# comprna/radian

Hardware: AMD Instinct MI355X
Metric: signal samples/s basecalled (chunk=1024, beam=10) (higher is better)
Workload: dtype f32

## Files before the change

### include/radian_hip.h

```cpp
#ifndef RADIAN_HIP_H
#define RADIAN_HIP_H

#include <stddef.h>
#include <stdint.h>

#ifdef __cplusplus
extern "C" {
#endif

#define RD_OK 0
#define RD_ERR_ARG (-1)
#define RD_ERR_HIP (-2)
#define RD_ERR_STATE (-3)
#define RD_ERR_NOMEM (-4)
#define RD_ERR_RCCL (-5)
#define RD_ERR_FORMAT (-6)
#define RD_ERR_IO (-7)
#define RD_LEN_MISSING_CONTEXT (-1)

typedef struct rd_ctx rd_ctx;

const char* rd_last_error(void);
int rd_version(void);
int rd_device_count(int* n);
int rd_decode_max_width(void);
int rd_decode_lane_width(void);

int rd_create(int device_id, rd_ctx** out);
int rd_destroy(rd_ctx* ctx);
int rd_sync(rd_ctx* ctx);
int rd_set_precision(rd_ctx* ctx, int mode);

typedef struct rd_weights_header {
    uint32_t magic;
    uint32_t version;
    uint32_t nb_filters;
    uint32_t kernel_size;
    uint32_t relu_units;
    uint32_t n_classes;
    uint32_t n_blocks;
    uint32_t dilations[16];
    uint32_t n_floats;
} rd_weights_header;
int rd_load_weights(rd_ctx* ctx, const void* blob, size_t nbytes);

int rd_load_lm(rd_ctx* ctx, const double* table, int k);
int rd_load_lm_absent(rd_ctx* ctx, int k);
int rd_load_lm_hashed(rd_ctx* ctx, const double* table, int table_order, int context_len);
int rd_set_logits(rd_ctx* ctx, int mode);
int rd_set_decode_partition(rd_ctx* ctx, int cus_per_xcd);
int rd_set_decode_math(rd_ctx* ctx, int mode);
int rd_set_head_pack(rd_ctx* ctx, int on);
int rd_head_pack_active(rd_ctx* ctx);
int64_t rd_head_pack_tiles(rd_ctx* ctx);
int rd_set_conv_slab(rd_ctx* ctx, int on);
int rd_conv_slab_active(rd_ctx* ctx);
int64_t rd_conv_slab_tiles(rd_ctx* ctx);

int rd_forward(rd_ctx* ctx, const float* windows, int n_windows, int chunk_len, float* probs);

int rd_assemble(rd_ctx* ctx, const float* probs, int n_windows, int chunk_len, int pad, int step, double* out,
                int64_t out_cap, int64_t* n_rows, int* is_f64);

int rd_decode_batch(rd_ctx* ctx, const void* probs, int prob_is_f64, const int64_t* seq_off, const int32_t* seq_len,
                    int n_seq, int beam_width, int use_lm, double s_thr, double r_thr, uint8_t* labels_out,
                    const int64_t* label_off, int32_t* label_len, double* best_score);

int rd_basecall_chunk(rd_ctx* ctx, const float* windows, int n_windows, int chunk_len, const int32_t* valid_len,
                      int beam_width, uint8_t* labels_out, int32_t* label_len);

int rd_basecall_global(rd_ctx* ctx, const float* windows, int chunk_len, int step, const int32_t* read_win_off,
                       const int32_t* pad, int n_reads, int beam_width, int use_lm, double s_thr, double r_thr,
                       uint8_t* labels_out, const int64_t* label_off, int32_t* label_len);

int rd_count_windows(int64_t n_samples, int chunk_len, int step);
int rd_basecall_reads_chunk(rd_ctx* ctx, const float* signal, const int64_t* read_off, int n_reads, int chunk_len,
                            int step, int beam_width, uint8_t* labels_out, int32_t* label_len);
int rd_basecall_reads_global(rd_ctx* ctx, const float* signal, const int64_t* read_off, int n_reads, int chunk_len,
                             int step, int beam_width, int use_lm, double s_thr, double r_thr, uint8_t* labels_out,
                             const int64_t* label_off, int32_t* label_len);

int rd_normalise_reads(rd_ctx* ctx, const int16_t* raw, const int64_t* read_off, int n_reads, int outlier_clip,
                       float* norm_out , int32_t* status);
int rd_basecall_raw_chunk(rd_ctx* ctx, const int16_t* raw, const int64_t* read_off, int n_reads, int outlier_clip,
                          int chunk_len, int step, int beam_width, uint8_t* labels_out, int32_t* label_len, int32_t* status);
int rd_basecall_raw_global(rd_ctx* ctx, const int16_t* raw, const int64_t* read_off, int n_reads, int outlier_clip,
                           int chunk_len, int step, int beam_width, int use_lm, double s_thr, double r_thr,
                           uint8_t* labels_out, const int64_t* label_off, int32_t* label_len, int32_t* status);

int rd_dev_alloc(rd_ctx* ctx, size_t bytes, void** d_ptr);
// ... 333 lines not shown
```

### radian_amd/_lib.py

```python
import ctypes
import os

HERE = os.path.dirname(os.path.abspath(__file__))
LIB_PATH = os.environ.get("RADIAN_HIP_LIB") or os.path.join(HERE, "libradian_hip.so")

c_i = ctypes.c_int
c_i32p = ctypes.POINTER(ctypes.c_int32)
c_i64 = ctypes.c_int64
c_i64p = ctypes.POINTER(ctypes.c_int64)
c_d = ctypes.c_double
c_dp = ctypes.POINTER(ctypes.c_double)
c_fp = ctypes.POINTER(ctypes.c_float)
c_u8p = ctypes.POINTER(ctypes.c_uint8)
c_u32 = ctypes.c_uint32
c_u64 = ctypes.c_uint64
c_vp = ctypes.c_void_p
c_sz = ctypes.c_size_t

SIGNATURES = {
    "rd_last_error": (ctypes.c_char_p, []),
    "rd_version": (c_i, []),
    "rd_device_count": (c_i, [ctypes.POINTER(c_i)]),
    "rd_decode_max_width": (c_i, []),
    "rd_decode_lane_width": (c_i, []),
    "rd_create": (c_i, [c_i, ctypes.POINTER(c_vp)]),
    "rd_destroy": (c_i, [c_vp]),
    "rd_sync": (c_i, [c_vp]),
    "rd_set_precision": (c_i, [c_vp, c_i]),
    "rd_load_weights": (c_i, [c_vp, c_vp, c_sz]),
    "rd_load_lm": (c_i, [c_vp, c_vp, c_i]),
    "rd_load_lm_absent": (c_i, [c_vp, c_i]),
    "rd_load_lm_hashed": (c_i, [c_vp, c_vp, c_i, c_i]),
    "rd_set_logits": (c_i, [c_vp, c_i]),
    "rd_set_decode_math": (c_i, [c_vp, c_i]),
    "rd_set_head_pack": (c_i, [c_vp, c_i]),
    "rd_head_pack_active": (c_i, [c_vp]),
    "rd_head_pack_tiles": (c_i64, [c_vp]),
    "rd_set_conv_slab": (c_i, [c_vp, c_i]),
    "rd_conv_slab_active": (c_i, [c_vp]),
    "rd_conv_slab_tiles": (c_i64, [c_vp]),
    "rd_set_decode_partition": (c_i, [c_vp, c_i]),
    "rd_forward": (c_i, [c_vp, c_vp, c_i, c_i, c_vp]),
    "rd_assemble": (c_i, [c_vp, c_vp, c_i, c_i, c_i, c_i, c_vp, c_i64, c_i64p, ctypes.POINTER(c_i)]),
    "rd_decode_batch": (c_i, [c_vp, c_vp, c_i, c_vp, c_vp, c_i, c_i, c_i, c_d, c_d, c_vp, c_vp, c_vp, c_vp]),
    "rd_basecall_chunk": (c_i, [c_vp, c_vp, c_i, c_i, c_vp, c_i, c_vp, c_vp]),
    "rd_basecall_global": (c_i, [c_vp, c_vp, c_i, c_i, c_vp, c_vp, c_i, c_i, c_i, c_d, c_d, c_vp, c_vp, c_vp]),
    "rd_count_windows": (c_i, [c_i64, c_i, c_i]),
    "rd_basecall_reads_chunk": (c_i, [c_vp, c_vp, c_vp, c_i, c_i, c_i, c_i, c_vp, c_vp]),
    "rd_basecall_reads_global": (c_i, [c_vp, c_vp, c_vp, c_i, c_i, c_i, c_i, c_i, c_d, c_d, c_vp, c_vp, c_vp]),
    "rd_basecall_reads_chunk_resident": (c_i, [c_vp, c_vp, c_vp, c_i, c_i, c_i, c_i, c_vp, c_vp]),
    "rd_basecall_reads_global_resident": (c_i, [c_vp, c_vp, c_vp, c_i, c_i, c_i, c_i, c_i, c_d, c_d, c_vp, c_vp, c_vp]),
    "rd_pipe_submit_reads": (c_i, [c_vp, c_vp, c_vp, c_i, c_i, c_i, c_i, c_vp, c_vp]),
    "rd_pipe_submit_reads_global": (c_i, [c_vp, c_vp, c_vp, c_i, c_i, c_i, c_i, c_i, c_d, c_d, c_vp, c_vp, c_vp]),
    "rd_pipe_submit_raw_global": (c_i, [c_vp, c_vp, c_vp, c_i, c_i, c_i, c_i, c_i, c_i, c_d, c_d, c_vp, c_vp, c_vp, c_vp]),
    "rd_pipe_submit_raw_chunk": (c_i, [c_vp, c_vp, c_vp, c_i, c_i, c_i, c_i, c_i, c_vp, c_vp, c_vp]),
    "rd_pipe_progress": (c_i, [c_vp, c_i64, c_i64p]),
    "rd_pipe_submitted": (c_i, [c_vp, c_i64p]),
    "rd_normalise_reads": (c_i, [c_vp, c_vp, c_vp, c_i, c_i, c_vp, c_vp]),
    "rd_basecall_raw_chunk": (c_i, [c_vp, c_vp, c_vp, c_i, c_i, c_i, c_i, c_i, c_vp, c_vp, c_vp]),
    "rd_basecall_raw_global": (c_i, [c_vp, c_vp, c_vp, c_i, c_i, c_i, c_i, c_i, c_i, c_d, c_d, c_vp, c_vp, c_vp, c_vp]),
    "rd_stitch_chunk": (c_i, [c_vp, c_vp, c_i, c_vp, c_i, c_vp, c_vp, c_vp, c_i]),
    "rd_fast5_open": (c_i, [ctypes.c_char_p, ctypes.POINTER(c_vp)]),
    "rd_fast5_open_mem": (c_i, [c_vp, c_sz, ctypes.POINTER(c_vp)]),
    "rd_fast5_close": (None, [c_vp]),
    "rd_fast5_count": (c_i, [c_vp, c_i64p]),
    "rd_fast5_lengths": (c_i, [c_vp, c_i64, c_i64, c_vp]),
    "rd_fast5_read_batch": (c_i, [c_vp, c_i64, c_i64, c_vp, c_i64, c_vp, c_vp, c_i]),
    "rd_lm_json_probe": (c_i, [c_vp, ctypes.c_size_t, ctypes.POINTER(c_i)]),
    "rd_lm_json_fill": (c_i, [c_vp, ctypes.c_size_t, c_i, c_vp, ctypes.POINTER(ctypes.c_int64), ctypes.POINTER(ctypes.c_int64)]),
    "rd_lm_json_write": (c_i, [ctypes.c_char_p, c_vp, c_i, c_i64p, c_i64p]),
    "rd_fasta_scan": (c_i, [c_vp, c_sz, c_i, ctypes.c_char_p, c_vp, c_vp, c_vp]),
    "rd_lm_build": (c_i, [c_vp, c_vp, c_vp, c_i64, c_i, c_i, c_i, c_d, c_d, c_i64, c_vp, c_vp, c_vp]),
    "rd_lm_score": (c_i, [c_vp, c_vp, c_vp, c_i64, c_i, c_d, c_i64, c_vp, c_dp]),
# ... 132 lines not shown
```

### radian_amd/backend.py

```python
import ctypes

import numpy as np

from . import _lib
from .weights import pack_blob, DEFAULT_DILATIONS

RD_TIMER_CONV, RD_TIMER_DECODE, RD_TIMER_HEAD, RD_TIMER_IN = 0, 1, 2, 3


class RadianHipError(RuntimeError):
    pass


def lib_path():
    return _lib.LIB_PATH


def _p(a):
    return None if a is None else a.ctypes.data_as(ctypes.c_void_p)


MISSING_CONTEXT = -1


# ... 972 lines not shown
            raise ValueError(f"LM table must be [4^{table_order},4], got {table.shape}")
        self._check(self._L.rd_load_lm_hashed(self._h, _p(table), int(table_order), int(context_len)))
        self.lm_k = context_len

    def set_logits(self, mode):
        self._check(self._L.rd_set_logits(self._h, {"f32": 0, "f16": 1}[mode] if isinstance(mode, str) else int(mode)))

    def set_trie_budget(self, nbytes):
        self._check(self._L.rd_set_trie_budget(self._h, int(nbytes)))

    def set_conv_fuse(self, on):
        self._check(self._L.rd_set_conv_fuse(self._h, 1 if on else 0))

    def set_head_pack(self, on):
        self._check(self._L.rd_set_head_pack(self._h, 1 if on else 0))

    def head_pack_active(self):
        return bool(self._L.rd_head_pack_active(self._h))

    def head_pack_tiles(self):
        return int(self._L.rd_head_pack_tiles(self._h))

    def set_conv_slab(self, on):
        self._check(self._L.rd_set_conv_slab(self._h, 1 if on else 0))

    def conv_slab_active(self):
        return bool(self._L.rd_conv_slab_active(self._h))

    def conv_slab_tiles(self):
        return int(self._L.rd_conv_slab_tiles(self._h))

    def set_decode_form(self, form):
        self._check(self._L.rd_set_decode_form(self._h, {"auto": 0, "waves": 1, "lanes": 2, "two": 3, "one": 4, "queue": 5}[form] if isinstance(form, str) else int(form)))

    def set_decode_partition(self, cus_per_xcd):
        self._check(self._L.rd_set_decode_partition(self._h, int(cus_per_xcd)))

    def set_decode_math(self, mode):
        self._check(self._L.rd_set_decode_math(self._h, {"fast": 0, "glibc": 1}[mode] if isinstance(mode, str) else int(mode)))

    def forward(self, windows):
        windows = np.ascontiguousarray(windows, dtype=np.float32)
        if windows.ndim != 2:
            raise ValueError("windows must be [n_windows, chunk_len]")
        n, T = windows.shape
        probs = np.empty((n, T, 5), dtype=np.float32)
        self._check(self._L.rd_forward(self._h, _p(windows), n, T, _p(probs)))
        return probs

    def assemble(self, probs, pad, step):
        probs = np.ascontiguousarray(probs, dtype=np.float32)
        nW, T, _ = probs.shape
        cap = (nW - 1) * step + T
        out = np.empty((max(cap, 1), 5), dtype=np.float64)
        n_rows = ctypes.c_int64(0)
        is64 = ctypes.c_int(0)
        self._check(self._L.rd_assemble(self._h, _p(probs), nW, T, int(pad), int(step), _p(out), out.shape[0],
                                        ctypes.byref(n_rows), ctypes.byref(is64)))
        out = out[: n_rows.value]
        return out if is64.value else out.astype(np.float32)

    def forward_reads(self, signals, chunk_len, step):
        flat, off = self._pack_reads(signals)
        nws = [self.count_windows(off[r + 1] - off[r], chunk_len, step) for r in range(len(signals))]
        tot = int(sum(nws))
        out = np.zeros((tot, chunk_len, 5), dtype=np.float32)
# ... 790 lines not shown
```

### radian_amd/csrc/common.h

```cpp
#pragma once
#include <hip/hip_runtime.h>
#include <stdint.h>
#include <stddef.h>
#include <string>
#include <vector>

#include "carve.h"
#include "polya_rules.h"

#define RD_OK 0
#define RD_ERR_ARG (-1)
#define RD_ERR_HIP (-2)
#define RD_ERR_STATE (-3)
#define RD_ERR_NOMEM (-4)
#define RD_ERR_RCCL (-5)

void rd_set_error(const char* fmt, ...);

#define RD_HIP(expr)                                                                                   \
    do {                                                                                               \
        hipError_t _e = (expr);                                                                        \
        if (_e != hipSuccess) {                                                                        \
            rd_set_error("%s:%d: %s failed: %s", __FILE__, __LINE__, #expr, hipGetErrorString(_e));   \
            return RD_ERR_HIP;                                                                         \
// ... 127 lines not shown
struct TileLists {
    const TileDesc* d[RD_MAX_LAYERS];
    int n[RD_MAX_LAYERS];
    int64_t rows[RD_MAX_LAYERS];
    const TileDesc* head_segs[RD_MAX_LAYERS];
    PackLayer pack[RD_MAX_LAYERS];
    int slab[RD_MAX_LAYERS];
    int slab_stream[RD_MAX_LAYERS];
};

struct KernelTimer {
    bool enabled = false;
    std::vector<hipEvent_t> starts, stops;
    size_t used = 0;
    double flops = 0.0;
    double bytes = 0.0;
    std::vector<double> each_flops;
    std::vector<int> each_tag;
};

constexpr int RD_MAX_LANES = 4;
struct FwdLane {
    hipStream_t st = nullptr;
    DevBuf act[3];
    hipEvent_t done = nullptr;
};

struct rd_ctx {
    int device = 0;
    int n_cu = 256;
    int precision = 0;
    int decode_form = 0;
    int decode_math = 1;
    int conv_fuse = 1;
    int64_t packed_tiles = 0;
    int head_pack = 1;
    int conv_slab = 1;
    int64_t slab_tiles = 0;
    int conv_shape = 0;
    int logits_f16 = 0;
    hipStream_t stream = nullptr;
    hipStream_t stream_hi = nullptr;
    hipEvent_t ev_chain = nullptr;
    Model model;
    LM lm;
    DevBuf ws_tiles, ws_raw;
    int tiles_nW = -1, tiles_T = -1;
    int tiles_slab = 0;
    FwdLane lanes[2 * RD_MAX_LANES];
    int part_mode = -1;
    int part_cus = 0;
    DevBuf ws_in, ws_probs, ws_mat, ws_seq, ws_nodes_child, ws_nodes_back, ws_labels, ws_misc;
    DevBuf ws_queue;
    DevBuf ws_wide, ws_wide_slot;
    DevBuf ws_align;
    DevBuf ws_ctc;
    DevBuf ws_calign;
    DevBuf ws_events, ws_events_io;
    DevBuf ws_polya, ws_polya_io;
    DevBuf ws_segment;
    DevBuf ws_sim;
    DevBuf ws_eval, ws_eval_model;
    DevBuf ws_site;
    DevBuf ws_quant;
    DevBuf pileup_sites;
    DevBuf pileup_profile;
    DevBuf ws_pileup;
    int64_t pileup_n_sites = -1;
    int64_t pileup_pairs = 0;
    int64_t trie_budget = (int64_t)24 << 30;
    void* h_stage = nullptr;
    size_t h_stage_cap = 0;
    bool h_stage_busy = false;
    KernelTimer timer_conv, timer_decode, timer_head, timer_in;
    void* rccl = nullptr;
    void* rpipe = nullptr;
    int pipe_group = 4;
    int pipe_lanes = 2;
    void* plan_cache[2] = {nullptr, nullptr};
    void* train = nullptr;
    void* map = nullptr;
};

size_t rd_model_image_floats(int nblocks);
void rd_model_bind(Model& m);
int rd_model_refresh_split(rd_ctx* ctx);
// ... 102 lines not shown
```

### radian_amd/csrc/context.hip

```cpp
#include "common.h"
#include "budget.h"
#include "../../include/radian_hip.h"
#include "../../include/radian_hip_diag.h"

#include <algorithm>
#include <stdarg.h>
#include <stdio.h>
#include <string.h>

static thread_local char g_err[1024] = "";

void rd_set_error(const char* fmt, ...)
{
    va_list ap;
    va_start(ap, fmt);
    vsnprintf(g_err, sizeof(g_err), fmt, ap);
    va_end(ap);
}

extern "C" const char* rd_last_error(void) { return g_err; }
extern "C" int rd_version(void) { return 1; }

int DevBuf::reserve(size_t bytes)
{
// ... 131 lines not shown
    t.starts.clear();
    t.stops.clear();
    t.each_flops.clear();
    t.each_tag.clear();
    t.used = 0;
    t.enabled = false;
}

extern "C" int rd_destroy(rd_ctx* ctx)
{
    if (!ctx) return RD_OK;
    (void)hipSetDevice(ctx->device);
    if (ctx->stream) (void)hipStreamSynchronize(ctx->stream);
    rd_rccl_finalize(ctx);
    rd_rpipe_destroy(ctx);
    rd_plan_cache_destroy_internal(ctx);
    rd_train_destroy(ctx);
    rd_map_destroy(ctx);
    timer_free(ctx->timer_conv);
    timer_free(ctx->timer_decode);
    timer_free(ctx->timer_head);
    timer_free(ctx->timer_in);
    for (int i = 0; i < 2 * RD_MAX_LANES; i++) {
        FwdLane& L = ctx->lanes[i];
        if (i > 0 && L.st) {
            (void)hipStreamSynchronize(L.st);
            if (i >= RD_MAX_LANES) rd_masked_stream_release(L.st);
            else (void)hipStreamDestroy(L.st);
        }
        if (L.done) (void)hipEventDestroy(L.done);
        for (DevBuf& b : L.act) b.release();
    }
    DevBuf* bufs[] = {&ctx->ws_tiles, &ctx->ws_raw, &ctx->ws_in, &ctx->ws_probs, &ctx->ws_mat, &ctx->ws_seq,
                      &ctx->ws_nodes_child, &ctx->ws_nodes_back, &ctx->ws_wide, &ctx->ws_wide_slot, &ctx->ws_align, &ctx->ws_ctc, &ctx->ws_calign, &ctx->ws_events, &ctx->ws_events_io, &ctx->ws_polya, &ctx->ws_polya_io, &ctx->ws_segment, &ctx->ws_eval, &ctx->ws_eval_model, &ctx->ws_site, &ctx->ws_quant, &ctx->pileup_sites, &ctx->pileup_profile, &ctx->ws_pileup, &ctx->ws_sim, &ctx->ws_queue, &ctx->ws_labels, &ctx->ws_misc, &ctx->model.storage,
                      &ctx->lm.storage, &ctx->lm.gate_storage};
    for (DevBuf* b : bufs) b->release();
    if (ctx->h_stage) (void)hipHostFree(ctx->h_stage);
    if (ctx->stream_hi) {
        (void)hipStreamSynchronize(ctx->stream_hi);
        (void)hipStreamDestroy(ctx->stream_hi);
    }
    if (ctx->ev_chain) (void)hipEventDestroy(ctx->ev_chain);
    if (ctx->stream) (void)hipStreamDestroy(ctx->stream);
    delete ctx;
    return RD_OK;
}

extern "C" int rd_set_precision(rd_ctx* ctx, int mode)
{
    RD_REQUIRE(ctx, "rd_set_precision: null context");
    RD_REQUIRE(mode >= 0 && mode <= 2, "rd_set_precision: mode %d (0 = fp32 MFMA, 1 = split-f16 f16x3, 2 = three-term bf16x3)", mode);
    ctx->precision = mode;
    return RD_OK;
}

extern "C" int rd_sync(rd_ctx* ctx)
{
    RD_REQUIRE(ctx, "rd_sync: null context");
    return rd_sync_lanes(ctx);
}

extern "C" int rd_set_logits(rd_ctx* ctx, int mode)
{
    RD_REQUIRE(ctx, "rd_set_logits: null context");
    RD_REQUIRE(mode == 0 || mode == 1, "rd_set_logits: mode %d (0 = float32 rows, 1 = float16 rows)", mode);
    ctx->logits_f16 = mode;
    return RD_OK;
}

extern "C" int rd_set_decode_form(rd_ctx* ctx, int form)
{
    RD_REQUIRE(ctx, "rd_set_decode_form: null context");
    RD_REQUIRE(form >= 0 && form <= 5, "rd_set_decode_form: form %d (0 = per launch, 1 = waves per sequence, 2 = candidates per lane, 3 = W <= 12: two sequences per "
               "wave, 4 = one, 5 = work queue)", form);
    ctx->decode_form = form;
    return RD_OK;
}

extern "C" int rd_set_trie_budget(rd_ctx* ctx, int64_t bytes)
{
    RD_REQUIRE(ctx, "rd_set_trie_budget: null context");
    RD_REQUIRE(bytes >= 0, "rd_set_trie_budget: negative budget");
    ctx->trie_budget = bytes ? bytes : (int64_t)24 << 30;
    return RD_OK;
}

extern "C" int rd_set_conv_shape(rd_ctx* ctx, int shape)
{
    RD_REQUIRE(ctx, "rd_set_conv_shape: null context");
    RD_REQUIRE(shape == 0 || shape == 1, "rd_set_conv_shape: shape %d (0 = 128-row tiles, two workgroups per CU; 1 = 256-row tiles, one workgroup per CU)", shape);
    ctx->conv_shape = shape;
    return RD_OK;
}

extern "C" int rd_set_conv_fuse(rd_ctx* ctx, int on)
{
    RD_REQUIRE(ctx, "rd_set_conv_fuse: null context");
    RD_REQUIRE(on == 0 || on == 1, "rd_set_conv_fuse: %d (1 = block 0's first conv inside its second, 0 = its own kernel)", on);
    ctx->conv_fuse = on;
    return RD_OK;
}

extern "C" int rd_set_head_pack(rd_ctx* ctx, int on)
{
    RD_REQUIRE(ctx, "rd_set_head_pack: null context");
    RD_REQUIRE(on == 0 || on == 1, "rd_set_head_pack: %d (1 = window heads as packed classes without their zero-padding taps, 0 = as head tiles)", on);
    ctx->head_pack = on;
    return RD_OK;
// ... 160 lines not shown
```

### radian_amd/csrc/decode.hip

```cpp
#include "common.h"
#include "glibc_math.h"
#include "glibc_tables.h"

#include <math.h>
#include <stdlib.h>

#include "decode_common.h"

namespace {

struct __attribute__((aligned(16))) Beam {
    double ptot, pb;
    double pnb;
    int last, len;
    int node;
    unsigned hist;
    unsigned hprev;
    int pad1;
    int child[4];
};
static_assert(sizeof(Beam) == 64, "Beam is one 64-B LDS record");

template <int R, int NW>
struct Cfg {
// ... 2 lines not shown
};
template <>
struct Cfg<2, 4> {
    static constexpr int WM = 64;
};


template <int NW>
__device__ __forceinline__ void seq_sync()
{
    if constexpr (NW == 1) {
        wave_sync();
    } else {
        __builtin_amdgcn_fence(__ATOMIC_RELEASE, "wavefront");
        asm volatile("s_waitcnt lgkmcnt(0)\n\ts_barrier" ::: "memory");
        __builtin_amdgcn_fence(__ATOMIC_ACQUIRE, "wavefront");
    }
}

template <typename PT, int R, int NW, bool LM, bool HC, bool GX>
__device__ __forceinline__ void beam_search_body(const DecodeArgs& a, const int seq)
{
    static_assert(LM || !HC, "hashed contexts only exist with an LM");
    constexpr int WM = Cfg<R, NW>::WM;
    constexpr int TPB = 64 * NW;
    constexpr int NS = R * NW;
    constexpr int KG = R == 1 ? 16 : 4;
    constexpr int SEG = 64 + KG;
    constexpr int HB = (WM + 63) / 64;
    constexpr int LOG_TN = WM > 128 ? 12 : WM > 64 ? 11 : R * NW <= 2 ? 9 : 10;
    constexpr int TN = 1 << LOG_TN;
    constexpr int SB = WM > 128 ? 9 : 8;
    constexpr int SMASK = (1 << SB) - 1;
    static_assert(WM <= 64 * HB && HB <= 4 && WM <= 256, "the kept beams fit the lanes of one wave, up to four times; a table entry holds a slot in 8 bits");
    static_assert(HB == 1 || !HC, "hashed contexts exist for up to 64 beams");
    const int tid = threadIdx.x;
    const int lane = tid & 63;
    const int wv = NW == 1 ? 0 : __builtin_amdgcn_readfirstlane(tid >> 6);
    const int T = a.seq_len[seq];
    const PT* __restrict__ probs = (const PT*)a.probs;
    const int64_t row_a = a.seq_off[seq];
    const int64_t row_b = a.seq_off2 ? a.seq_off2[seq] : row_a;
    const int split = a.seq_off2 ? a.seq_split[seq] : 0;
    int4* __restrict__ childtab = a.childtab + a.node_off[seq];
    int* __restrict__ backptr = a.backptr + a.node_off[seq];
    const int W = a.W;
    const unsigned ctx_mask = LM ? ((a.k >= 16) ? 0xffffffffu : ((1u << (2 * a.k)) - 1u)) : 0u;

    __shared__ Beam st[2][WM];
    constexpr int SCR = 5 * WM, KEYS = NS * SEG;
    __shared__ __attribute__((aligned(16))) double dbuf[NW == 1 ? (SCR > KEYS ? SCR : KEYS) : SCR + KEYS + (SCR & 1)];
    double* const cpy_pnb = dbuf;
    double* const cpy_pb = dbuf + WM;
    double* const mb_v = dbuf + 2 * WM;
    double* const mP = dbuf + 3 * WM;
    double* const mQ = dbuf + 4 * WM;
    double* const keyC = NW == 1 ? dbuf : dbuf + SCR + (SCR & 1);
    __shared__ int mb_q[WM];
    __shared__ int d_sel[WM], newslot[WM];
    __shared__ unsigned claims[WM];
    __shared__ double lp[64][5];
    __shared__ double praw[LM ? 64 : 1][5];
    __shared__ double sent[LM ? 64 : 1];
    __shared__ int seg_s[NS], seg_v[NS], mflag[NW];
    __shared__ unsigned tab[TN];
    constexpr bool GXL = GX && R == 1;
    __shared__ uint64_t gx_lds[GXL ? 256 : 1];
    if constexpr (GXL)
        for (int i = tid; i < 256; i += TPB) gx_lds[i] = g_gm_exp_tab[i];
    const uint64_t* const gx_exp = GXL ? gx_lds : g_gm_exp_tab;
    __shared__ __attribute__((aligned(16))) unsigned ring[2][HC ? WM : 1][16];

    for (int i = tid; i < TN; i += TPB) tab[i] = i == 0 ? 0u : 0xffffffffu;
    if (tid == 0) {
        Beam& b = st[0][0];
        b.ptot = 0.0;
        b.pb = 0.0;
        b.pnb = -INFINITY;
        b.last = -1;
        b.len = 0;
        b.node = 0;
        b.hist = 0u;
        b.hprev = 0u;
        b.pad1 = 0;
        for (int c = 0; c < 4; c++) b.child[c] = 0;
        childtab[0] = make_int4(0, 0, 0, 0);
        backptr[0] = 0;
    }
    int nb = 1;
    int next_id = 1;
    int cur = 0;
    bool missed = false;
    seq_sync<NW>();

    for (int t0 = 0; t0 < T; t0 += 64) {
        if (NW == 1 || wv == 0) {
            const int t = t0 + lane;
            if (t < T) {
                const PT* __restrict__ prow = probs + ((t < split ? row_a : row_b) + t) * 5;
                double s4 = 0.0;
#pragma unroll 1
                for (int c = 0; c < 5; c++) {
                    const double pc = (double)prow[c];
                    lp[lane][c] = safe_log<GX>(pc);
                    if constexpr (LM) {
                        praw[lane][c] = pc;
                        if (c < 4) s4 = c == 0 ? pc : s4 + pc;
                    }
                }
                if constexpr (LM) {
                    const double s = s4;
                    double ent = 0.0;
                    bool any = false;
#pragma unroll 1
                    for (int c = 0; c < 4; c++) {
                        const double pc = praw[lane][c];
                        double n;
                        if (s == 0.0) n = pc;
                        else if constexpr (sizeof(PT) == 4) n = (double)((float)pc / (float)s);
                        else n = pc / s;
                        if (n > 0) {
                            double v = n * log_m<GX>(n);
                            ent = any ? ent + v : v;
                            any = true;
                        }
                    }
                    sent[lane] = any ? -ent : 0.0;
                }
            }
        }
        seq_sync<NW>();

        const int tend = (T - t0) < 64 ? (T - t0) : 64;
        for (int tt = 0; tt < tend; tt++) {
            const Beam* os = st[cur];
            Beam* __restrict__ ns = st[cur ^ 1];
            const int ncand = 5 * nb;

            bool valid[R], is_copy[R];
            int bi[R], kk[R], pj[R], dcopy[R], xch[R];
            double c_ptot[R], c_pnb[R], c_pb[R];
            const double lp_blank = lp[tt][4];
            bool s_open = false;
            if constexpr (LM) s_open = __builtin_amdgcn_readfirstlane((int)(sent[tt] > a.s_thr)) != 0;
            const double ptot_last = os[nb - 1].ptot;
            int myn[HB];
            if constexpr (HB == 1) {
                myn[0] = os[lane < nb ? lane : 0].node;
            } else {
#pragma unroll
                for (int h = 0; h < HB; h++) myn[h] = os[lane + 64 * h < nb ? lane + 64 * h : 0].node;
            }
            double2 pp[R];
            double pnb_i[R];
            int2 ll[R];
            int chx[R];
#pragma unroll
            for (int s = 0; s < R; s++) {
                const int q = s * TPB + tid;
                valid[s] = q < ncand;
                const int i = valid[s] ? q / 5 : 0;
                const int k = q - 5 * (q / 5);
                bi[s] = i;
                kk[s] = k;
                is_copy[s] = k == 0;
                pp[s] = *(const double2*)&os[i].ptot;
                pnb_i[s] = os[i].pnb;
                ll[s] = *(const int2*)&os[i].last;
                int4 c4 = *(const int4*)&os[i].child[0];
                asm("" : "+v"(c4.x), "+v"(c4.y), "+v"(c4.z), "+v"(c4.w));
// ... 85 lines not shown
#pragma unroll
                    for (int s = 0; s < R; s++)
                        if (xch[s] != 0 && nj == xch[s]) pj[s] = j;
                }
            }
            bool any_merge = false;
#pragma unroll
            for (int s = 0; s < R; s++) any_merge |= __any(pj[s] >= 0);
            if constexpr (NW > 1) {
                if (lane == 0) mflag[wv] = any_merge ? 1 : 0;
            }
            seq_sync<NW>();
            if constexpr (NW > 1) {
                int m = 0;
#pragma unroll
                for (int w = 0; w < NW; w++) m |= mflag[w];
                any_merge = __builtin_amdgcn_readfirstlane(m) != 0;
            }

#pragma unroll
            for (int s = 0; s < R; s++) {
                const bool mext = pj[s] >= 0;
                const double cp = cpy_pnb[mext ? pj[s] : 0];
                const double x = mext ? cp : c_pb[s];
                const double y = mext ? c_ptot[s] : c_pnb[s];
                const double r = GX ? lae_gx(x, y, gx_exp) : lae(x, y);
                c_ptot[s] = is_copy[s] ? r : c_ptot[s];
                if (mext) {
                    mb_q[pj[s]] = s * TPB + tid;
                    mb_v[pj[s]] = c_ptot[s];
                    mQ[pj[s]] = r;
                }
            }
            if (any_merge) {
                seq_sync<NW>();
#pragma unroll
                for (int s = 0; s < R; s++) {
                    const int qe = mb_q[bi[s]];
                    const double mv = mb_v[bi[s]];
                    const bool m = valid[s] & is_copy[s] & (qe >= 0);
                    const double r = GX ? lae_gx(c_ptot[s], m ? mv : -INFINITY, gx_exp) : lae(c_ptot[s], m ? mv : -INFINITY);
                    if (m) mP[bi[s]] = r;
                }
                seq_sync<NW>();
#pragma unroll
                for (int s = 0; s < R; s++) {
                    const int q = s * TPB + tid;
                    const int j = is_copy[s] ? bi[s] : (pj[s] >= 0 ? pj[s] : 0);
                    const int qe = mb_q[j];
                    const double P = mP[j], Q = mQ[j], cb = cpy_pb[j];
                    const bool merged = valid[s] & (is_copy[s] ? qe >= 0 : pj[s] >= 0);
                    const int qother = is_copy[s] ? qe : 5 * j;
                    const bool mk = merged & (q < qother);
                    const bool mke = mk & !is_copy[s];
                    c_ptot[s] = mk ? P : c_ptot[s];
                    c_pnb[s] = mk ? Q : c_pnb[s];
                    c_pb[s] = mke ? cb : c_pb[s];
                    dcopy[s] = mke ? j : dcopy[s];
                    valid[s] = valid[s] & (!merged | mk);
                }
            }

            double key[R];
            bool surv[R];
            int lidx[R], scnt[R], vcnt[R];
            const double tau = (nb == W) ? ptot_last + lp_blank : -INFINITY;
#pragma unroll
            for (int s = 0; s < R; s++) {
                key[s] = valid[s] ? c_ptot[s] : __builtin_nan("");
                surv[s] = valid[s] && key[s] >= tau;
                const unsigned long long mv = __ballot(valid[s]), ms = __ballot(surv[s]);
                vcnt[s] = __popcll(mv);
                scnt[s] = __popcll(ms);
                lidx[s] = (int)__builtin_amdgcn_mbcnt_hi((unsigned)(ms >> 32), __builtin_amdgcn_mbcnt_lo((unsigned)ms, 0u));
                double* kseg = keyC + (s * NW + wv) * SEG;
                if (lane < KG) kseg[scnt[s] + lane] = -INFINITY;
                if (surv[s]) kseg[lidx[s]] = key[s];
                if constexpr (NW > 1) {
                    if (lane == 0) {
                        seg_s[s * NW + wv] = scnt[s];
                        seg_v[s * NW + wv] = vcnt[s];
                    }
                }
            }
            seq_sync<NW>();
            int segn[NS];
            int nvalid = 0;
#pragma unroll
            for (int g = 0; g < NS; g++) {
                if constexpr (NW > 1) {
                    segn[g] = __builtin_amdgcn_readfirstlane(seg_s[g]);
                    nvalid += __builtin_amdgcn_readfirstlane(seg_v[g]);
                } else {
                    segn[g] = scnt[g];
                    nvalid += vcnt[g];
                }
            }
            int rank[R];
#pragma unroll
            for (int s = 0; s < R; s++) rank[s] = 0;
#pragma unroll
            for (int g = 0; g < NS; g++) {
                const double* kseg = keyC + g * SEG;
                for (int j = 0; j < segn[g]; j += KG) {
                    double2 kq[KG / 2];
#pragma unroll
                    for (int u = 0; u < KG / 2; u++) kq[u] = *(const double2*)&kseg[j + 2 * u];
#pragma unroll
                    for (int u = 0; u < KG / 4; u++)
#pragma unroll
                        for (int s = 0; s < R; s++)
                            rank[s] = count4_gt(rank[s], kq[2 * u].x, kq[2 * u].y, kq[2 * u + 1].x, kq[2 * u + 1].y, key[s]);
                }
            }
            const int nb_new = nvalid < W ? nvalid : W;

            if constexpr (NW == 1 && R == 1) {
                const bool top = surv[0] && rank[0] < W;
                const unsigned long long m_top = __ballot(top), m_same = __ballot(top && dcopy[0] >= 0 && rank[0] == dcopy[0]);
                if (m_top == m_same && __popcll(m_top) == nb && nb_new == nb) {
                    if (top) {
                        Beam* const here = st[cur] + rank[0];
                        *(double2*)&here->ptot = make_double2(c_ptot[0], c_pb[0]);
                        here->pnb = c_pnb[0];
                    }
                    wave_sync();
                    continue;
                }
            }

            auto scatter = [&]() {
#pragma unroll
                for (int s = 0; s < R; s++) {
                    if (surv[s] && rank[s] < W) {
                        const int r = rank[s];
                        *(double2*)&ns[r].ptot = make_double2(c_ptot[s], c_pb[s]);
                        ns[r].pnb = c_pnb[s];
                        d_sel[r] = (dcopy[s] & SMASK) | (bi[s] << SB) | (kk[s] << (2 * SB));
                        atomicAdd(&claims[r], 1u);
                        if (dcopy[s] >= 0) newslot[dcopy[s]] = r;
                    }
                }
            };
            scatter();
            seq_sync<NW>();
            unsigned n_claims[HB], my_tn2[HB];
            int sel[HB], my_newslot[HB];
            bool claim_bad;
            if constexpr (HB == 1) {
                n_claims[0] = claims[lane < nb_new ? lane : 0];
                sel[0] = d_sel[lane < nb_new ? lane : 0];
                my_newslot[0] = newslot[lane < nb ? lane : 0];
                my_tn2[0] = tab[myn[0] & (TN - 1)];
                asm volatile("" : "+v"(sel[0]), "+v"(my_newslot[0]), "+v"(my_tn2[0]));
                claim_bad = (lane < nb_new) & (n_claims[0] != 1u);
            } else {
                claim_bad = false;
// ... 144 lines not shown
                                ch.x = __hip_atomic_load(cp + 0, __ATOMIC_RELAXED, __HIP_MEMORY_SCOPE_AGENT);
                                ch.y = __hip_atomic_load(cp + 1, __ATOMIC_RELAXED, __HIP_MEMORY_SCOPE_AGENT);
                                ch.z = __hip_atomic_load(cp + 2, __ATOMIC_RELAXED, __HIP_MEMORY_SCOPE_AGENT);
                                ch.w = __hip_atomic_load(cp + 3, __ATOMIC_RELAXED, __HIP_MEMORY_SCOPE_AGENT);
                            }
                            asm volatile("s_waitcnt vmcnt(0)" : "+v"(ch.x), "+v"(ch.y), "+v"(ch.z), "+v"(ch.w));
                        }
                        if (act) {
                            const int new_node = is_ext ? my_node : meta.x;
                            *(int2*)&ns[bl].last = make_int2(is_ext ? cl : sl2.x, is_ext ? sl2.y + 1 : sl2.y);
                            const unsigned h_new = ((unsigned)meta.y << 2) | (unsigned)cl;
                            if constexpr (LM) {
                                if (a.lm_missing && is_ext && sl2.y + 1 >= a.k && t0 + tt + 1 < T) {
                                    const unsigned cx = h_new & ctx_mask;
                                    missed |= ((a.lm_missing[cx >> 5] >> (cx & 31)) & 1u) != 0u;
                                }
                            }
                            *(int4*)&ns[bl].node = make_int4(new_node, is_ext ? (int)h_new : meta.y, meta.z, 0);
                            *(int4*)&ns[bl].child[0] = make_int4(is_ext ? ch.x : chs.x, is_ext ? ch.y : chs.y, is_ext ? ch.z : chs.z, is_ext ? ch.w : chs.w);
                            tab[new_node & (TN - 1)] = (((unsigned)new_node >> LOG_TN) << 8) | (unsigned)bl;
                        }
                        fresh_h[h] = fresh;
                        ps_h[h] = ps;
                        cl_h[h] = cl;
                        node_h[h] = my_node;
                    }
#pragma unroll
                    for (int h = 0; h < HB; h++)
                        if (fresh_h[h] && ps_h[h] >= 0) ns[ps_h[h]].child[cl_h[h]] = node_h[h];
                }
            }
            nb = nb_new;
            cur ^= 1;
            seq_sync<NW>();
        }
    }

    int tid_end = tid;
    asm volatile("" : "+v"(tid_end));
    const bool any_missed = LM && __any(missed);
    if (tid_end == 0) {
        __builtin_amdgcn_s_waitcnt(0);
        const char* ka = (const char*)__builtin_amdgcn_kernarg_segment_ptr();
        asm volatile("" : "+s"(ka));
        const DecodeArgs* ap = (const DecodeArgs*)ka;
        const Beam& fs = st[cur][0];
        int n = fs.node;
        const int len = fs.len;
        uint8_t* out = ap->labels + ap->label_off[seq];
        for (int p = len - 1; p >= 0; p--) {
            const int bp = __hip_atomic_load(&backptr[n], __ATOMIC_RELAXED, __HIP_MEMORY_SCOPE_AGENT);
            out[p] = (uint8_t)(bp & 3);
            n = bp >> 2;
        }
        ap->label_len[seq] = any_missed ? -1 : len;
        if (ap->best_score) ap->best_score[seq] = fs.ptot;
    }
}


template <typename PT, int R, int NW, bool LM, bool HC, bool GX>
__global__ __launch_bounds__(64 * NW) void beam_search_kernel(DecodeArgs a)
{
    beam_search_body<PT, R, NW, LM, HC, GX>(a, (int)blockIdx.x);
}

template <typename PT, int R, int NW, bool LM, bool HC, bool GX>
__global__ __launch_bounds__(64 * NW) void beam_search_queue_kernel(DecodeArgs a, int n_seq, int* counter)
{
    __shared__ int s_next;
    for (;;) {
        if (threadIdx.x == 0) s_next = atomicAdd(counter, 1);
        __syncthreads();
        const int seq = __builtin_amdgcn_readfirstlane(s_next);
        __syncthreads();
        if (seq >= n_seq) return;
        beam_search_body<PT, R, NW, LM, HC, GX>(a, seq);
        __syncthreads();
    }
}


template <typename PT, bool LM, bool GX, int R>
__global__ __launch_bounds__(64) void beam_search2_kernel(DecodeArgs a, int n_seq)
{
    constexpr int WM = R == 1 ? 6 : 12;
    constexpr int TS = 32;
    constexpr int KG = R == 1 ? 16 : 8;
    constexpr int SEG = 32 + KG;
// ... 583 lines not shown
        if (!ctx->lm.loaded) {
            rd_set_error("decode with use_lm=1 but no LM table loaded (rd_load_lm)");
            return RD_ERR_STATE;
        }
        int rc = ensure_lm_gate(ctx, r_thr, st);
        if (rc) return rc;
    }
    if (ctx->ws_nodes_child.reserve((size_t)total_nodes * sizeof(int4))) return RD_ERR_NOMEM;
    if (ctx->ws_nodes_back.reserve((size_t)total_nodes * sizeof(int))) return RD_ERR_NOMEM;
    DecodeArgs a;
    a.probs = d_probs;
    a.seq_off = d_seq_off;
    a.seq_off2 = d_seq_off2;
    a.seq_split = d_seq_split;
    a.seq_len = d_seq_len;
    a.node_off = d_node_off;
    a.label_off = d_label_off;
    a.W = W;
    a.glibc_math = ctx->decode_math;
    a.lm_table = use_lm ? ctx->lm.table : nullptr;
    a.lm_gate = use_lm ? ctx->lm.gate_bits : nullptr;
    a.lm_missing = (use_lm && ctx->lm.sparse && !ctx->lm.hashed) ? ctx->lm.d_missing : nullptr;
    a.k = use_lm ? ctx->lm.k : 0;
    a.hashed = use_lm ? ctx->lm.hashed : 0;
    a.tmask = use_lm ? (unsigned)(((size_t)1 << (2 * ctx->lm.table_order)) - 1) : 0u;
    a.bk = 1u;
    for (int i = 0; use_lm && i < ctx->lm.k; i++) a.bk *= kHashB;
    a.s_thr = s_thr;
    a.childtab = ctx->ws_nodes_child.as<int4>();
    a.backptr = ctx->ws_nodes_back.as<int>();
    a.labels = d_labels;
    a.label_len = d_label_len;
    a.best_score = d_best_score;
    KernelTimer& tm = ctx->timer_decode;
    if (tm.enabled && tm.used < tm.starts.size()) RD_HIP(hipEventRecord(tm.starts[tm.used], st));
    int rc;
    if (ctx->decode_form == 5 && queue_wave_slots == 0) queue_wave_slots = 16;
    if (queue_wave_slots > 0 && W <= kMaxW4 && !(use_lm && a.hashed)) {
        if (ctx->ws_queue.reserve(256)) return RD_ERR_NOMEM;
        RD_HIP(hipMemsetAsync(ctx->ws_queue.p, 0, 4, st));
        int* counter = ctx->ws_queue.as<int>();
        rc = ptype == 1 ? launch_queue_pt<double>(st, a, n_seq, use_lm != 0, queue_wave_slots, counter)
             : ptype == 2 ? launch_queue_pt<_Float16>(st, a, n_seq, use_lm != 0, queue_wave_slots, counter)
                          : launch_queue_pt<float>(st, a, n_seq, use_lm != 0, queue_wave_slots, counter);
    } else
    rc = W > kMaxW4 ? rd_decode_wide_launch(ctx, st, &a, ptype, n_seq, total_nodes, use_lm != 0)
             : ptype == 1 ? launch_pt<double>(st, a, n_seq, use_lm != 0, n_simd, ctx->decode_form)
             : ptype == 2 ? launch_pt<_Float16>(st, a, n_seq, use_lm != 0, n_simd, ctx->decode_form) : launch_pt<float>(st, a, n_seq, use_lm != 0, n_simd, ctx->decode_form);
    if (rc) return rc;
    if (tm.enabled && tm.used < tm.starts.size()) {
        RD_HIP(hipEventRecord(tm.stops[tm.used], st));
        tm.used++;
    }
    return RD_OK;
}
```

### radian_amd/csrc/decode_common.h

```cpp
#pragma once
#include "common.h"
#include "glibc_math.h"
#include "glibc_tables.h"

#include <math.h>

namespace {


__device__ const uint64_t g_gm_exp_tab[256] = RD_GLIBC_EXP_TAB;
__device__ const uint64_t g_gm_log_tab[256] = RD_GLIBC_LOG_TAB;

constexpr unsigned kHashB = 0x9E3779B1u;
constexpr double kLogE2 = 0.693147180559945309417232121458176568;

#pragma clang fp contract(off)
__device__ __forceinline__ double horner10(double q, double x, double c0, double c1, double c2, double c3, double c4, double c5,
                                           double c6, double c7, double c8, double c9)
{
    asm("v_fma_f64 %0, %0, %1, %2\n\tv_fma_f64 %0, %0, %1, %3\n\tv_fma_f64 %0, %0, %1, %4\n\tv_fma_f64 %0, %0, %1, %5\n\t"
        "v_fma_f64 %0, %0, %1, %6\n\tv_fma_f64 %0, %0, %1, %7\n\tv_fma_f64 %0, %0, %1, %8\n\tv_fma_f64 %0, %0, %1, %9\n\t"
        "v_fma_f64 %0, %0, %1, %10\n\tv_fma_f64 %0, %0, %1, %11"
        : "+v"(q)
        : "v"(x), "s"(c0), "s"(c1), "s"(c2), "s"(c3), "s"(c4), "s"(c5), "s"(c6), "s"(c7), "s"(c8), "s"(c9));
// ... 92 lines not shown

template <bool GX>
__device__ __forceinline__ double log_m(double x)
{
    if constexpr (GX) return gm_log(x, g_gm_log_tab);
    else return log(x);
}
template <bool GX>
__device__ __forceinline__ double safe_log(double x) { return (x > 0.0 && x <= 1.79769313486231570815e+308) ? log_m<GX>(x) : -INFINITY; }

struct DecodeArgs {
    const void* probs;
    const int64_t* seq_off;
    const int64_t* seq_off2;
    const int32_t* seq_split;
    const int32_t* seq_len;
    const int64_t* node_off;
    const int64_t* label_off;
    int W;
    int glibc_math;
    const double* lm_table;
    const uint32_t* lm_gate;
    const uint32_t* lm_missing;
    int k;
    int hashed;
    unsigned tmask;
    unsigned bk;
    double s_thr;
    int4* childtab;
    int* backptr;
    uint8_t* labels;
    int32_t* label_len;
    double* best_score;
};

}
```

Before: 28.02 million.

## Reuse previous scores-only step structure in beam decode to skip candidate selection

Adds a decode 'chain' mode, on by default for single-wave, non-LM decode. After a step that only updated scores, the per-lane candidate, merge and holder decisions are packed into one register word. The next step replays that structure and checks that the beam ordering still holds, skipping candidate generation, ranking and merge discovery. If the check fails it falls back to the full step, and the kernel gains diagnostic counters for held and fallen-back steps. This trades extra register state and a validation pass per step against fewer full top-W selections.

```diff
diff --git a/include/radian_hip.h b/include/radian_hip.h
--- a/include/radian_hip.h
+++ b/include/radian_hip.h
@@ -56,6 +56,8 @@
 int rd_set_conv_slab(rd_ctx* ctx, int on);
 int rd_conv_slab_active(rd_ctx* ctx);
 int64_t rd_conv_slab_tiles(rd_ctx* ctx);
+int rd_set_decode_chain(rd_ctx* ctx, int on);
+int rd_diag_decode_chain_steps(rd_ctx* ctx, int64_t* out);
 
 int rd_forward(rd_ctx* ctx, const float* windows, int n_windows, int chunk_len, float* probs);
 
diff --git a/radian_amd/_lib.py b/radian_amd/_lib.py
--- a/radian_amd/_lib.py
+++ b/radian_amd/_lib.py
@@ -39,6 +39,8 @@
     "rd_set_conv_slab": (c_i, [c_vp, c_i]),
     "rd_conv_slab_active": (c_i, [c_vp]),
     "rd_conv_slab_tiles": (c_i64, [c_vp]),
+    "rd_set_decode_chain": (c_i, [c_vp, c_i]),
+    "rd_diag_decode_chain_steps": (c_i, [c_vp, c_i64p]),
     "rd_set_decode_partition": (c_i, [c_vp, c_i]),
     "rd_forward": (c_i, [c_vp, c_vp, c_i, c_i, c_vp]),
     "rd_assemble": (c_i, [c_vp, c_vp, c_i, c_i, c_i, c_i, c_vp, c_i64, c_i64p, ctypes.POINTER(c_i)]),
diff --git a/radian_amd/backend.py b/radian_amd/backend.py
--- a/radian_amd/backend.py
+++ b/radian_amd/backend.py
@@ -1028,6 +1028,14 @@
 
     def set_decode_form(self, form):
         self._check(self._L.rd_set_decode_form(self._h, {"auto": 0, "waves": 1, "lanes": 2, "two": 3, "one": 4, "queue": 5}[form] if isinstance(form, str) else int(form)))
+
+    def set_decode_chain(self, on):
+        self._check(self._L.rd_set_decode_chain(self._h, 1 if on else 0))
+
+    def decode_chain_steps(self):
+        out = (ctypes.c_int64 * 2)()
+        self._check(self._L.rd_diag_decode_chain_steps(self._h, out))
+        return int(out[0]), int(out[1])
 
     def set_decode_partition(self, cus_per_xcd):
         self._check(self._L.rd_set_decode_partition(self._h, int(cus_per_xcd)))
diff --git a/radian_amd/csrc/common.h b/radian_amd/csrc/common.h
--- a/radian_amd/csrc/common.h
+++ b/radian_amd/csrc/common.h
@@ -183,6 +183,8 @@
     int precision = 0;
     int decode_form = 0;
     int decode_math = 1;
+    int decode_chain = 1;
+    bool chain_armed = false;
     int conv_fuse = 1;
     int64_t packed_tiles = 0;
     int head_pack = 1;
@@ -203,6 +205,7 @@
     int part_cus = 0;
     DevBuf ws_in, ws_probs, ws_mat, ws_seq, ws_nodes_child, ws_nodes_back, ws_labels, ws_misc;
     DevBuf ws_queue;
+    DevBuf ws_chain;
     DevBuf ws_wide, ws_wide_slot;
     DevBuf ws_align;
     DevBuf ws_ctc;
diff --git a/radian_amd/csrc/context.hip b/radian_amd/csrc/context.hip
--- a/radian_amd/csrc/context.hip
+++ b/radian_amd/csrc/context.hip
@@ -187,7 +187,7 @@
         for (DevBuf& b : L.act) b.release();
     }
     DevBuf* bufs[] = {&ctx->ws_tiles, &ctx->ws_raw, &ctx->ws_in, &ctx->ws_probs, &ctx->ws_mat, &ctx->ws_seq,
-                      &ctx->ws_nodes_child, &ctx->ws_nodes_back, &ctx->ws_wide, &ctx->ws_wide_slot, &ctx->ws_align, &ctx->ws_ctc, &ctx->ws_calign, &ctx->ws_events, &ctx->ws_events_io, &ctx->ws_polya, &ctx->ws_polya_io, &ctx->ws_segment, &ctx->ws_eval, &ctx->ws_eval_model, &ctx->ws_site, &ctx->ws_quant, &ctx->pileup_sites, &ctx->pileup_profile, &ctx->ws_pileup, &ctx->ws_sim, &ctx->ws_queue, &ctx->ws_labels, &ctx->ws_misc, &ctx->model.storage,
+                      &ctx->ws_nodes_child, &ctx->ws_nodes_back, &ctx->ws_wide, &ctx->ws_wide_slot, &ctx->ws_align, &ctx->ws_ctc, &ctx->ws_calign, &ctx->ws_events, &ctx->ws_events_io, &ctx->ws_polya, &ctx->ws_polya_io, &ctx->ws_segment, &ctx->ws_eval, &ctx->ws_eval_model, &ctx->ws_site, &ctx->ws_quant, &ctx->pileup_sites, &ctx->pileup_profile, &ctx->ws_pileup, &ctx->ws_sim, &ctx->ws_queue, &ctx->ws_chain, &ctx->ws_labels, &ctx->ws_misc, &ctx->model.storage,
                       &ctx->lm.storage, &ctx->lm.gate_storage};
     for (DevBuf* b : bufs) b->release();
     if (ctx->h_stage) (void)hipHostFree(ctx->h_stage);
@@ -229,6 +229,33 @@
     RD_REQUIRE(form >= 0 && form <= 5, "rd_set_decode_form: form %d (0 = per launch, 1 = waves per sequence, 2 = candidates per lane, 3 = W <= 12: two sequences per "
                "wave, 4 = one, 5 = work queue)", form);
     ctx->decode_form = form;
+    return RD_OK;
+}
+
+extern "C" int rd_set_decode_chain(rd_ctx* ctx, int on)
+{
+    RD_REQUIRE(ctx, "rd_set_decode_chain: null context");
+    RD_REQUIRE(on == 0 || on == 1, "rd_set_decode_chain: %d (1 = a step after a scores-only step reuses its structure, 0 = every step is a full one)", on);
+    ctx->decode_chain = on;
+    return RD_OK;
+}
+
+extern "C" int rd_diag_decode_chain_steps(rd_ctx* ctx, int64_t* out)
+{
+    RD_REQUIRE(ctx && out, "rd_diag_decode_chain_steps: null argument");
+    RD_HIP(hipSetDevice(ctx->device));
+    RD_HIP(hipDeviceSynchronize());
+    out[0] = out[1] = 0;
+    if (!ctx->chain_armed) {
+        if (ctx->ws_chain.reserve(2 * sizeof(unsigned long long))) return RD_ERR_NOMEM;
+    } else {
+        unsigned long long h[2];
+        RD_HIP(hipMemcpy(h, ctx->ws_chain.p, sizeof(h), hipMemcpyDeviceToHost));
+        out[0] = (int64_t)h[0];
+        out[1] = (int64_t)h[1];
+    }
+    RD_HIP(hipMemset(ctx->ws_chain.p, 0, 2 * sizeof(unsigned long long)));
+    ctx->chain_armed = true;
     return RD_OK;
 }
 
diff --git a/radian_amd/csrc/decode.hip b/radian_amd/csrc/decode.hip
--- a/radian_amd/csrc/decode.hip
+++ b/radian_amd/csrc/decode.hip
@@ -58,6 +58,7 @@
     constexpr int TN = 1 << LOG_TN;
     constexpr int SB = WM > 128 ? 9 : 8;
     constexpr int SMASK = (1 << SB) - 1;
+    constexpr bool CH = NW == 1 && R == 1 && !LM;
     static_assert(WM <= 64 * HB && HB <= 4 && WM <= 256, "the kept beams fit the lanes of one wave, up to four times; a table entry holds a slot in 8 bits");
     static_assert(HB == 1 || !HC, "hashed contexts exist for up to 64 beams");
     const int tid = threadIdx.x;
@@ -117,6 +118,10 @@
     int next_id = 1;
     int cur = 0;
     bool missed = false;
+    const bool chain_on = CH && a.chain != 0;
+    bool held = false, h_anymerge = false;
+    unsigned h_pack = 0u;
+    int n_held = 0, n_fell = 0;
     seq_sync<NW>();
 
     for (int t0 = 0; t0 < T; t0 += 64) {
@@ -162,6 +167,72 @@
             const Beam* os = st[cur];
             Beam* __restrict__ ns = st[cur ^ 1];
             const int ncand = 5 * nb;
+
+            if constexpr (CH) {
+                if (held) {
+                    const bool h_cw = h_pack & 1u, h_iscopy = h_pack & 2u, h_cneg = h_pack & 4u, h_selpb = h_pack & 8u, h_mext = h_pack & 16u;
+                    const bool h_m2 = h_pack & 32u, h_mk = h_pack & 64u, h_mke = h_pack & 128u, h_holder = h_pack & 256u, h_skip = h_pack & 512u;
+                    const int h_bi = (h_pack >> 10) & 15, h_j = (h_pack >> 14) & 15, h_c = (h_pack >> 18) & 7, h_hold = (h_pack >> 21) & 15,
+                              h_ref = (h_pack >> 25) & 15;
+                    {
+                        const double lpb = lp[tt][4];
+                        const double2 pp = *(const double2*)&os[h_bi].ptot;
+                        const double pnb_i = os[h_bi].pnb;
+                        double lpc = lp[tt][h_c];
+                        lpc = h_cneg ? -INFINITY : lpc;
+                        const double pnb_c = h_cneg ? -INFINITY : pnb_i + lpc;
+                        const double pb_c = pp.x + lpb;
+                        const double v = (h_selpb ? pp.y : pp.x) + lpc;
+                        double e_pnb = h_iscopy ? pnb_c : v;
+                        double e_pb = h_iscopy ? pb_c : -INFINITY;
+                        double e_ptot = h_iscopy ? 0.0 : v;
+                        double x = e_pb, y = e_pnb;
+                        if (h_anymerge) {
+                            if (h_cw) {
+                                cpy_pnb[h_bi] = pnb_c;
+                                cpy_pb[h_bi] = pb_c;
+                            }
+                            wave_sync();
+                            const double cp = cpy_pnb[h_j];
+                            x = h_mext ? cp : x;
+                            y = h_mext ? e_ptot : y;
+                        }
+                        const double r1 = GX ? lae_gx(x, y, gx_exp) : lae(x, y);
+                        e_ptot = h_iscopy ? r1 : e_ptot;
+                        if (h_anymerge) {
+                            if (h_mext) {
+                                mb_v[h_j] = e_ptot;
+                                mQ[h_j] = r1;
+                            }
+                            wave_sync();
+                            const double mv = mb_v[h_bi];
+                            const double r2 = GX ? lae_gx(e_ptot, h_m2 ? mv : -INFINITY, gx_exp) : lae(e_ptot, h_m2 ? mv : -INFINITY);
+                            if (h_m2) mP[h_bi] = r2;
+                            wave_sync();
+                            const double P = mP[h_j], Q = mQ[h_j], cb = cpy_pb[h_j];
+                            e_ptot = h_mk ? P : e_ptot;
+                            e_pnb = h_mk ? Q : e_pnb;
+                            e_pb = h_mke ? cb : e_pb;
+                        }
+                        if (h_holder) dbuf[h_hold] = e_ptot;
+                        wave_sync();
+                        const double kref = dbuf[h_ref];
+                        const bool ok = h_skip | (e_ptot < kref);
+                        if (!__any(!ok)) {
+                            if (h_holder) {
+                                Beam* const here = st[cur] + h_hold;
+                                *(double2*)&here->ptot = make_double2(e_ptot, e_pb);
+                                here->pnb = e_pnb;
+                            }
+                            wave_sync();
+                            n_held++;
+                            continue;
+                        }
+                        n_fell++;
+                        held = false;
+                    }
+                }
+            }
 
             bool valid[R], is_copy[R];
             int bi[R], kk[R], pj[R], dcopy[R], xch[R];
@@ -313,6 +384,7 @@
                     mQ[pj[s]] = r;
                 }
             }
+            bool f_m2 = false, f_mk = false, f_mke = false;
             if (any_merge) {
                 seq_sync<NW>();
 #pragma unroll
@@ -322,6 +394,7 @@
                     const bool m = valid[s] & is_copy[s] & (qe >= 0);
                     const double r = GX ? lae_gx(c_ptot[s], m ? mv : -INFINITY, gx_exp) : lae(c_ptot[s], m ? mv : -INFINITY);
                     if (m) mP[bi[s]] = r;
+                    if constexpr (CH) f_m2 = m;
                 }
                 seq_sync<NW>();
 #pragma unroll
@@ -339,6 +412,10 @@
                     c_pb[s] = mke ? cb : c_pb[s];
                     dcopy[s] = mke ? j : dcopy[s];
                     valid[s] = valid[s] & (!merged | mk);
+                    if constexpr (CH) {
+                        f_mk = mk;
+                        f_mke = mke;
+                    }
                 }
             }
 
@@ -404,6 +481,26 @@
                         Beam* const here = st[cur] + rank[0];
                         *(double2*)&here->ptot = make_double2(c_ptot[0], c_pb[0]);
                         here->pnb = c_pnb[0];
+                    }
+                    if constexpr (CH) {
+                        if (chain_on && nb == W) {
+                            const int last0 = ll[0].x;
+                            const int c0 = is_copy[0] ? last0 : kk[0] - 1;
+                            const bool holder = valid[0] && dcopy[0] >= 0;
+                            const int hold = holder ? dcopy[0] : 0;
+                            const bool skip = !valid[0] || (holder && hold == 0);
+                            const int ref = holder && hold > 0 ? hold - 1 : W - 1;
+                            const int j0 = is_copy[0] ? bi[0] : (pj[0] >= 0 ? pj[0] : 0);
+                            unsigned pk = ((tid < ncand) & is_copy[0] ? 1u : 0u)
+                                          | (is_copy[0] ? 2u : 0u) | (c0 < 0 ? 4u : 0u) | (last0 == kk[0] - 1 ? 8u : 0u) | (pj[0] >= 0 ? 16u : 0u)
+                                          | (f_m2 ? 32u : 0u) | (f_mk ? 64u : 0u) | (f_mke ? 128u : 0u) | (holder ? 256u : 0u) | (skip ? 512u : 0u)
+                                          | ((unsigned)bi[0] << 10) | ((unsigned)j0 << 14) | ((unsigned)(c0 < 0 ? 0 : c0) << 18) | ((unsigned)hold << 21)
+                                          | ((unsigned)ref << 25);
+                            asm volatile("" : "+v"(pk));
+                            h_pack = pk;
+                            h_anymerge = any_merge;
+                            held = true;
+                        }
                     }
                     wave_sync();
                     continue;
@@ -614,6 +711,7 @@
             }
             nb = nb_new;
             cur ^= 1;
+            if constexpr (CH) held = false;
             seq_sync<NW>();
         }
     }
@@ -637,6 +735,12 @@
         }
         ap->label_len[seq] = any_missed ? -1 : len;
         if (ap->best_score) ap->best_score[seq] = fs.ptot;
+        if constexpr (CH) {
+            if (ap->chain_cnt) {
+                atomicAdd(&ap->chain_cnt[0], (unsigned long long)n_held);
+                atomicAdd(&ap->chain_cnt[1], (unsigned long long)n_fell);
+            }
+        }
     }
 }
 
@@ -1286,6 +1390,8 @@
     a.labels = d_labels;
     a.label_len = d_label_len;
     a.best_score = d_best_score;
+    a.chain = ctx->decode_chain;
+    a.chain_cnt = ctx->chain_armed ? ctx->ws_chain.as<unsigned long long>() : nullptr;
     KernelTimer& tm = ctx->timer_decode;
     if (tm.enabled && tm.used < tm.starts.size()) RD_HIP(hipEventRecord(tm.starts[tm.used], st));
     int rc;
diff --git a/radian_amd/csrc/decode_common.h b/radian_amd/csrc/decode_common.h
--- a/radian_amd/csrc/decode_common.h
+++ b/radian_amd/csrc/decode_common.h
@@ -148,6 +148,8 @@
     uint8_t* labels;
     int32_t* label_len;
     double* best_score;
+    int chain;
+    unsigned long long* chain_cnt;
 };
 
 }
```

Result: no change. 28.29 million, median of 6 (+1.0%).
